# muzishen/IMAGDressing

Measured on AMD Instinct MI355X. Metric: 512x512 50-step images/sec (whole node), higher is better.
Workload: dtype bf16

## Files before the change

imagdressing_amd/_lib.py:

```python
from __future__ import annotations

import ctypes as C
import os

_HERE = os.path.dirname(os.path.abspath(__file__))
LIB_PATH = os.environ.get("IMD_LIB_PATH") or os.path.join(_HERE, "libimagdressing_hip.so")

ABI_VERSION = 9

u16p = C.POINTER(C.c_uint16)
f32p = C.POINTER(C.c_float)


class _Sized(C.Structure):

    def __init__(self, *args, **kw):
        super().__init__(*args, **kw)
        self.struct_bytes = C.sizeof(self)


class HeadsDest(C.Structure):
    _fields_ = [("ptr", C.c_void_p), ("kind", C.c_int), ("DP", C.c_int), ("L", C.c_int), ("scale", C.c_float)]


# ... 74 lines not shown

SYMBOLS = {
    "imd_abi_version": (C.c_int, []),
    "imd_last_error": (C.c_char_p, []),
    "imd_device_check": (C.c_int, [C.c_int]),
    "imd_conv_gemm": (C.c_int, [C.POINTER(ConvGemmParams), C.c_int, C.c_void_p]),
    "imd_conv_gemm_auto_cfg": (C.c_int, [C.c_int, C.c_int]),
    "imd_conv_gemm_auto_split": (C.c_int, [C.c_int, C.c_int, C.c_int, C.c_int]),
    "imd_attention": (C.c_int, [C.POINTER(AttnParams), C.c_void_p]),
    "imd_attention_dup_supported": (C.c_int, [C.c_int, C.c_int, C.c_int]),
    "imd_attention_phase_split_supported": (C.c_int, [C.c_int]),
    "imd_attention_fp8": (C.c_int, [C.POINTER(AttnParams), C.c_int, C.c_int, C.c_int, C.c_void_p]),
    "imd_attn_quantize_fp8": (C.c_int, [C.c_void_p, C.c_void_p, C.c_int, C.c_long, C.c_int, C.c_int, C.c_float, C.c_int, C.c_void_p]),
    "imd_set_tuning": (C.c_int, [C.c_int, C.c_int]),
    "imd_get_tuning": (C.c_int, [C.c_int]),
    "imd_attn_padded_dims": (C.c_int, [C.c_int, C.POINTER(C.c_int), C.POINTER(C.c_int)]),
    "imd_groupnorm": (C.c_int, [C.POINTER(GroupNormParams), C.c_void_p]),
    "imd_groupnorm_coeffs": (C.c_int, [C.POINTER(GroupNormParams), C.c_void_p, C.c_void_p, C.c_void_p]),
    "imd_conv_patch_supported": (C.c_int, [C.POINTER(ConvGemmParams)]),
    "imd_conv_patch2_supported": (C.c_int, [C.POINTER(ConvGemmParams)]),
    "imd_conv_patch3_supported": (C.c_int, [C.POINTER(ConvGemmParams)]),
    "imd_conv_patch4_supported": (C.c_int, [C.POINTER(ConvGemmParams)]),
    "imd_conv_img_supported": (C.c_int, [C.POINTER(ConvGemmParams)]),
    "imd_conv_patch_stats_parts": (C.c_int, [C.POINTER(ConvGemmParams)]),
    "imd_conv_gemm_stats_parts": (C.c_int, [C.POINTER(ConvGemmParams), C.c_int]),
    "imd_conv_gemm_gn_out_supported": (C.c_int, [C.POINTER(ConvGemmParams)]),
    "imd_row_linear_gn_in_supported": (C.c_int, [C.POINTER(ConvGemmParams), C.c_int]),
    "imd_gemm_dma_supported": (C.c_int, [C.POINTER(ConvGemmParams)]),
    "imd_row_linear": (C.c_int, [C.POINTER(ConvGemmParams), C.c_int, C.c_float, C.c_void_p]),
    "imd_row_linear_supported": (C.c_int, [C.POINTER(ConvGemmParams)]),
    "imd_ff_geglu": (C.c_int, [C.POINTER(FfParams), C.c_void_p]),
    "imd_text_xattn320": (C.c_int, [C.POINTER(XattnParams), C.c_void_p]),
    "imd_text_xattn320_supported": (C.c_int, [C.POINTER(XattnParams)]),
    "imd_groupnorm_workspace_floats": (C.c_int, [C.c_int, C.c_int, C.c_int, C.c_int]),
    "imd_layernorm": (C.c_int, [C.POINTER(LayerNormParams), C.c_void_p]),
    "imd_softmax_rows": (C.c_int, [C.c_void_p, C.c_int, C.c_void_p, C.c_int, C.c_int, C.c_int, C.c_int, C.c_void_p]),
    "imd_ddim_cfg_step": (C.c_int, [C.POINTER(DdimParams), C.c_void_p]),
    "imd_ddim_cfg_step_rows": (C.c_int, [C.POINTER(DdimParams), C.c_void_p, C.c_void_p]),
    "imd_timestep_embedding": (C.c_int, [C.c_void_p, C.c_void_p, C.c_int, C.c_int, C.c_void_p]),
    "imd_add": (C.c_int, [C.c_void_p, C.c_int, C.c_void_p, C.c_int, C.c_void_p, C.c_int, C.c_long, C.c_int, C.c_float, C.c_int, C.c_void_p]),
    "imd_embed_tokens": (C.c_int, [C.c_void_p, C.c_int, C.c_void_p, C.c_int, C.c_void_p, C.c_void_p, C.c_long, C.c_int, C.c_int, C.c_void_p]),
    "imd_vit_assemble": (C.c_int, [C.c_void_p, C.c_void_p, C.c_void_p, C.c_void_p, C.c_int, C.c_int, C.c_int, C.c_int, C.c_void_p]),
    "imd_lincomb": (C.c_int, [C.POINTER(C.c_void_p), C.POINTER(C.c_float), C.c_int, C.c_void_p, C.c_long, C.c_void_p]),
    "imd_copy2d": (C.c_int, [C.c_void_p, C.c_int, C.c_void_p, C.c_int, C.c_long, C.c_int, C.c_void_p]),
    "imd_concat2": (C.c_int, [C.c_void_p, C.c_int, C.c_void_p, C.c_int, C.c_void_p, C.c_void_p, C.c_long, C.c_long, C.c_int, C.c_void_p]),
    "imd_concat2_gn_stats": (C.c_int, [C.c_void_p, C.c_int, C.c_void_p, C.c_int, C.c_void_p, C.c_void_p, C.c_int, C.c_int, C.c_int, C.c_int,
                                       C.c_void_p, C.c_int, C.c_void_p]),
    "imd_groupnorm_parts": (C.c_int, [C.c_int, C.c_int, C.c_int]),
    "imd_f32_to_16": (C.c_int, [C.c_void_p, C.c_void_p, C.c_long, C.c_int, C.c_void_p]),
}

_lib = None


class ImdError(RuntimeError):
    pass


def load():
    global _lib
    if _lib is None:
        if not os.path.isfile(LIB_PATH):
            raise ImdError(
                f"{LIB_PATH} not found: build it with `python -c 'import __graft_entry__ as g; g.build()'` "
                "(or imagdressing_amd/csrc/build.sh).  imagdressing_amd has no CPU / torch fallback.")
        lib = C.CDLL(LIB_PATH)
# ... 13 lines not shown
```

imagdressing_amd/csrc/capi.cpp:

```cpp
#include <atomic>
#include <mutex>
#include <stdarg.h>
#include <stdio.h>
#include <string.h>

#include "imd_kernels.h"

namespace {
thread_local char g_err[512] = "";
}

int imd_set_error(const char* fmt, ...) {
    va_list ap;
    va_start(ap, fmt);
    vsnprintf(g_err, sizeof(g_err), fmt, ap);
    va_end(ap);
    return 1;
}

int imd_check_launch(const char* what) {
    hipError_t e = hipGetLastError();
    if (e != hipSuccess) return imd_set_error("%s: launch failed: %s", what, hipGetErrorString(e));
    return 0;
}
// ... 179 lines not shown
        IMD_REQUIRE(p->hC > 0 && p->hH > 0 && p->hD > 0 && p->hC == p->hH * p->hD && p->N % p->hC == 0 && p->N / p->hC <= 3 && p->hD % 8 == 0,
                    "row_linear: bad head split C=%d H=%d D=%d", p->hC, p->hH, p->hD);
        IMD_REQUIRE(!p->out_f32, "row_linear: head-split output excludes fp32 output");
    }
    IMD_REQUIRE(!ln || ln_eps > 0.f, "row_linear: LayerNorm needs eps > 0");
    if (p->K == 320 && p->N == 960 && p->mode == IMD_OUT_HEADS) {
        IMD_REQUIRE(p->gn_in_partial == nullptr, "row_linear: the fused q / k / v projection has no GroupNorm prologue (gn_in_*)");
        return imd_launch_row_qkv(*p, ln, ln_eps, (hipStream_t)stream);
    }
    if (p->K == 640) return imd_launch_row_linear_k640(*p, ln, ln_eps, (hipStream_t)stream);
    if (p->K == 1280) return imd_launch_row_linear_k1280(*p, ln, ln_eps, (hipStream_t)stream);
    return imd_launch_row_linear(*p, ln, ln_eps, (hipStream_t)stream);
}

int imd_ff_geglu(const imd_ff_params* p, void* stream) {
    IMD_REQUIRE(p != nullptr, "ff_geglu: null params");
    IMD_REQUIRE_SIZE(p, "ff_geglu");
    IMD_REQUIRE(p->x && p->w1 && p->b1 && p->w2 && p->b2 && p->out, "ff_geglu: null pointer");
    IMD_REQUIRE(!p->ln || p->ln_eps > 0.f, "ff_geglu: LayerNorm needs eps > 0");
    return imd_launch_ff_geglu(*p, (hipStream_t)stream);
}

int imd_text_xattn320_supported(const imd_xattn_params* p) {
    return (p && p->struct_bytes == sizeof(*p) && imd_text_xattn320_supported_of(*p)) ? 1 : 0;
}

int imd_text_xattn320(const imd_xattn_params* p, void* stream) {
    IMD_REQUIRE(p != nullptr, "text_xattn320: null params");
    IMD_REQUIRE_SIZE(p, "text_xattn320");
    IMD_REQUIRE(p->x && p->w && p->bq && p->bo && p->kv && p->out, "text_xattn320: null pointer");
    return imd_launch_text_xattn320(*p, (hipStream_t)stream);
}

int imd_layernorm(const imd_layernorm_params* p, void* stream) {
    IMD_REQUIRE(p != nullptr, "layernorm: null params");
    IMD_REQUIRE_SIZE(p, "layernorm");
    IMD_REQUIRE(p->x && p->y && p->gamma && p->beta, "layernorm: null pointer");
    return imd_launch_layernorm(*p, (hipStream_t)stream);
}

int imd_embed_tokens(const uint16_t* table, int vocab, const uint16_t* pos, int T, const int64_t* ids, uint16_t* out, long rows, int C,
                     int dtype, void* stream) {
    IMD_REQUIRE(table && pos && ids && out, "embed_tokens: null pointer");
    return imd_launch_embed_tokens(table, vocab, pos, T, ids, out, rows, C, dtype, (hipStream_t)stream);
}

int imd_vit_assemble(const uint16_t* patches, const uint16_t* cls, const uint16_t* pos, uint16_t* out, int B, int P, int C, int dtype,
                     void* stream) {
    IMD_REQUIRE(patches && cls && pos && out, "vit_assemble: null pointer");
    return imd_launch_vit_assemble(patches, cls, pos, out, B, P, C, dtype, (hipStream_t)stream);
}

int imd_lincomb(const float* const* xs, const float* coefs, int n, float* out, long numel, void* stream) {
    IMD_REQUIRE(xs && coefs && out, "lincomb: null pointer");
    return imd_launch_lincomb(xs, coefs, n, out, numel, (hipStream_t)stream);
}

int imd_softmax_rows(const float* s, int s_ld, uint16_t* p, int p_ld, int rows, int cols, int dtype, void* stream) {
    IMD_REQUIRE(s && p, "softmax_rows: null pointer");
    return imd_launch_softmax_rows(s, s_ld, p, p_ld, rows, cols, dtype, (hipStream_t)stream);
}

int imd_ddim_cfg_step(const imd_ddim_params* p, void* stream) {
    IMD_REQUIRE(p != nullptr, "ddim_cfg_step: null params");
    IMD_REQUIRE_SIZE(p, "ddim_cfg_step");
    IMD_REQUIRE(p->z && p->eps, "ddim_cfg_step: null pointer");
// ... 47 lines not shown
```

imagdressing_amd/csrc/conv_patch.hip:

```cpp
#include <type_traits>

#include "gemm_common.h"
#include "lds_dma.h"

namespace {

constexpr int TH = 8, TW = 16;
constexpr int PW = TW + 2, PH = TH + 2;
constexpr int NPIX = PH * PW;
constexpr int CK = 32;
constexpr int RSTR = CK * 2 + 16;
constexpr int BN = 128;
constexpr int A_BYTES = NPIX * RSTR;
constexpr int W_BYTES = BN * RSTR;
constexpr int MAIN_LDS = 2 * A_BYTES + 2 * W_BYTES;
constexpr int CLD = BN + 4;
constexpr int EROWS = 64;
constexpr int EPI_LDS = EROWS * CLD * 4;
constexpr int PATCH_LDS = MAIN_LDS > EPI_LDS ? MAIN_LDS : EPI_LDS;
constexpr int A_VECS = (NPIX * (CK / 8) + 255) / 256;
__device__ constexpr unsigned char kColPix[32] = {0, 1, 2, 3, 8, 9, 10, 11, 12, 13, 14, 15, 4, 5, 6, 7,
                                                  30, 31, 16, 17, 22, 23, 24, 25, 26, 27, 28, 29, 18, 19, 20, 21};
constexpr int W_VECS = BN * (CK / 8) / 256;

// ... 398 lines not shown
            float S = 0.f, Q = 0.f;
            for (int j = 0; j < CPR; ++j) {
                const int nj = n0 + 8 * j;
                if (nj >= p.N) break;
                const int gj = nj / cpg;
                if (gj == g || gj + 1 == g) {
                    const int o = (gj == g) ? 0 : 2;
                    for (int rl = 0; rl < 256 / CPR; ++rl) { S += red[(j + CPR * rl) * 4 + o]; Q += red[(j + CPR * rl) * 4 + o + 1]; }
                }
            }
            const int nparts = tiles_y * tiles_x * n_tiles;
            const int part = (ty * tiles_x + tx) * n_tiles + tile_n;
            float* dst = p.gn_stats_out + (((size_t)b * nparts + part) * G + g) * 2;
            dst[0] = S; dst[1] = Q;
        }
    }
    if (slab != nullptr && p.splitk_counters != nullptr) {
        if (splitk_last_arrival(p.splitk_counters, tile_id, p.split_k, tid)) {
            for (int ch = tid; ch < TH * TW * CPR; ch += 256) {
                const int q = ch / CPR, cc = (ch - q * CPR) * 8;
                const int oy = y0 + q / TW, ox = x0 + q % TW;
                const int n = n0 + cc;
                if (n >= p.N || oy >= H || ox >= W) continue;
                const int m = (b * H + oy) * W + ox;
                const int nv = (n + 8 <= p.N) ? 8 : 4;
                float v[8];
                splitk_sum8(p, m, n, nv, v);
                epilogue8<F16>(p, v, m, n, nv, HW);
            }
        }
    }
}

}

int imd_conv_patch_stats_parts_of(const ConvGemmParams& p) {
    if (!imd_conv_patch_supported(p) || p.split_k > 1 || p.out_f32 || p.gn_stats_groups <= 0 || p.gn_stats_groups > 64 ||
        p.N % p.gn_stats_groups || (p.N / p.gn_stats_groups) < 8)
        return 0;
    return ((p.Hout + TH - 1) / TH) * ((p.Wout + TW - 1) / TW) * ((p.N + BN - 1) / BN);
}

bool imd_conv_patch_supported(const ConvGemmParams& p) {
    const bool geom = p.ups ? (p.Hout == 2 * p.Hin && p.Wout == 2 * p.Win && p.gn_a == nullptr && !(g_gemm_flags & 512))
                            : (p.Hin == p.Hout && p.Win == p.Wout);
    return p.taps == 9 && p.stride == 1 && !p.pad_br_only && geom && p.Hout >= TH && p.Wout >= TW && (p.Cin % CK) == 0 &&
           p.mode == OUT_ROWMAJOR && p.act != ACT_GEGLU;
}

bool imd_conv_patch64_supported(const ConvGemmParams& p) {
    return imd_conv_patch_supported(p) && (p.Cin % 64) == 0 && p.gn_a == nullptr && !(g_gemm_flags & 512) && p.x_bytes < 0x80000000u && p.w_bytes < 0x80000000u;
}

int imd_launch_conv_patch64(const ConvGemmParams& p, hipStream_t s) {
    if (!imd_conv_patch64_supported(p)) return imd_set_error("conv_patch (128-byte rows): unsupported problem (needs 3x3 stride 1, H >= 8, W >= 16, Cin %% 64 == 0, operands < 2 GiB, no fused GroupNorm)");
    const bool h = p.dtype == IMD_DTYPE_F16;
    typedef void (*kern_t)(const ConvGemmParams);
    const kern_t kern = h ? conv3x3_patch_kernel<true, true, 64> : conv3x3_patch_kernel<false, true, 64>;
    if (int rc_attr = imd_lds_attr(reinterpret_cast<const void*>(kern), PD<64>::LDS, "conv_patch")) return rc_attr;
    const int B = p.M / (p.Hout * p.Wout);
    const long blocks = (long)B * ((p.Hout + TH - 1) / TH) * ((p.Wout + TW - 1) / TW) * ((p.N + BN - 1) / BN);
    hipLaunchKernelGGL(kern, dim3((unsigned)blocks, (unsigned)p.split_k), dim3(256), PD<64>::LDS, s, p);
    return imd_check_launch("conv_patch (128-byte rows)");
}

int imd_launch_conv_patch(const ConvGemmParams& p, hipStream_t s) {
// ... 15 lines not shown
```

imagdressing_amd/csrc/imd_kernels.h:

```cpp
#pragma once
#include <hip/hip_runtime.h>
#include <stdint.h>

#include "../../include/imagdressing_hip.h"

typedef uint16_t bf16_t;
typedef imd_heads_dest HeadsDest;
typedef imd_conv_gemm_params ConvGemmParams;
typedef imd_attn_params AttnParams;
typedef imd_groupnorm_params GroupNormParams;
typedef imd_layernorm_params LayerNormParams;
typedef imd_ddim_params DdimParams;

enum { ACT_NONE = IMD_ACT_NONE, ACT_SILU = IMD_ACT_SILU, ACT_GEGLU = IMD_ACT_GEGLU, ACT_GELU = IMD_ACT_GELU, ACT_QUICK_GELU = IMD_ACT_QUICK_GELU };
enum { OUT_ROWMAJOR = IMD_OUT_ROWMAJOR, OUT_HEADS = IMD_OUT_HEADS };

int imd_set_error(const char* fmt, ...);
int imd_check_launch(const char* what);
int imd_lds_attr(const void* kern, int bytes, const char* what);
int imd_cu_count8();

int imd_conv_gemm_choose_cfg(int M, int N);
int imd_conv_gemm_choose_split(int M, int N, int K, int cfg);
int imd_launch_conv_gemm(const ConvGemmParams& p, int cfg, hipStream_t s);
bool imd_conv_gemm_fill_extents(ConvGemmParams& p);
bool imd_conv_patch_supported(const ConvGemmParams& p);
bool imd_conv_patch2_supported(const ConvGemmParams& p);
int imd_launch_conv_patch2(const ConvGemmParams& p, hipStream_t s);
bool imd_conv_patch3_supported(const ConvGemmParams& p);
int imd_launch_conv_patch3(const ConvGemmParams& p, hipStream_t s);
bool imd_conv_patch4_supported(const ConvGemmParams& p);
int imd_launch_conv_patch4(const ConvGemmParams& p, hipStream_t s);
int imd_conv_patch3_stats_parts_of(const ConvGemmParams& p, int nw);
bool imd_conv_patch64_supported(const ConvGemmParams& p);
int imd_launch_conv_patch64(const ConvGemmParams& p, hipStream_t s);
bool imd_conv_img_supported(const ConvGemmParams& p);
int imd_launch_conv_img(const ConvGemmParams& p, hipStream_t s);
int imd_conv_patch_stats_parts_of(const ConvGemmParams& p);
int imd_conv_gemm_stats_parts_of(const ConvGemmParams& p, int cfg);
bool imd_conv_gemm_gn_out_supported_of(const ConvGemmParams& p, int cfg);
bool imd_row_linear_gn_in_supported_of(const ConvGemmParams& p, int cfg);
int imd_launch_conv_patch(const ConvGemmParams& p, hipStream_t s);
bool imd_row_linear_supported(const ConvGemmParams& p);
int imd_launch_row_linear(const ConvGemmParams& p, int ln, float ln_eps, hipStream_t s);
bool imd_row_linear_k640_supported(const ConvGemmParams& p);
int imd_launch_row_linear_k640(const ConvGemmParams& p, int ln, float ln_eps, hipStream_t s);
bool imd_row_linear_k1280_supported(const ConvGemmParams& p);
int imd_launch_row_linear_k1280(const ConvGemmParams& p, int ln, float ln_eps, hipStream_t s);
bool imd_row_qkv_supported(const ConvGemmParams& p);
int imd_launch_row_qkv(const ConvGemmParams& p, int ln, float ln_eps, hipStream_t s);
bool imd_gemm_dma_supported(const ConvGemmParams& p);
int imd_launch_gemm_dma(const ConvGemmParams& p, hipStream_t s);
int imd_launch_gemm_dma128(const ConvGemmParams& p, int stages, int bk, hipStream_t s);
int imd_launch_gemm_dma256(const ConvGemmParams& p, int form, hipStream_t s);
bool imd_conv_dma_supported(const ConvGemmParams& p);
int imd_launch_ff_geglu(const imd_ff_params& p, hipStream_t s);
bool imd_text_xattn320_supported_of(const imd_xattn_params& p);
int imd_launch_text_xattn320(const imd_xattn_params& p, hipStream_t s);
int imd_launch_attention(const AttnParams& p, hipStream_t s);
int imd_launch_attention_d40(const AttnParams& p, int variant, hipStream_t s);
int imd_launch_attention_fp8(const AttnParams& p, int eq, int ek, int ev, hipStream_t s);
int imd_launch_attn_quantize_fp8(const bf16_t* src, unsigned char* dst, int kind, long rows_or_groups, int LP, int exp2_scale,
                                 float pad_val, int dtype, hipStream_t s);
extern int g_attn_qw40;
extern int g_attn_xcd;
#ifdef IMD_ATTN_SWEEP
extern int g_attn_v80, g_attn_v160;
#endif
// ... 21 lines not shown
```

imagdressing_amd/ops.py:

```python
from __future__ import annotations

import functools
import ctypes as C
from typing import Dict, Optional, Sequence, Tuple

import torch

from . import _lib as L

ACT_NONE, ACT_SILU, ACT_GEGLU, ACT_GELU, ACT_QUICK_GELU = 0, 1, 2, 3, 4
bf16 = torch.bfloat16
f16 = torch.float16
DTYPE_CODE = {torch.bfloat16: 0, torch.float16: 1}


def _code(t: torch.Tensor, name: str = "tensor") -> int:
    try:
        return DTYPE_CODE[t.dtype]
    except KeyError:
        raise L.ImdError(f"{name}: expected a bfloat16 or float16 tensor, got {t.dtype}") from None


try:
    _raw_stream, _cur_dev = torch._C._cuda_getCurrentRawStream, torch._C._cuda_getDevice
# ... 575 lines not shown
    p.x, p.w, p.out = _dev(x, dt, "x"), _dev(packed["w"], dt, "w"), _dev(out, dt, "out")
    p.bq, p.bo, p.kv = _dev(packed["bq"], torch.float32, "bq"), _dev(packed["bo"], torch.float32, "bo"), _dev(kv_img, dt, "kv_img")
    p.M, p.C, p.heads, p.L = B * N, C_, XATTN_HEADS, int(Lk)
    p.rows_per_image, p.kv_bdiv, p.text_rows = N, int(kv_bdiv), kv_img.shape[0]
    p.x_ld = p.out_ld = C_
    p.q_scale = float(XATTN_D ** -0.5 * 1.4426950408889634 if q_scale is None else q_scale)
    p.ln_eps, p.dtype = float(ln_eps), _code(x, "x")
    _count("gemm_conv", 2 * 2.0 * B * N * C_ * C_)
    _count("attention", 4.0 * XATTN_HEADS * N * XATTN_D * B * Lk)
    L.check(L.load().imd_text_xattn320(C.byref(p), _stream()))
    return out


def conv2d_nhwc(x: torch.Tensor, w: torch.Tensor, bias=None, *, taps=9, stride=1, ups=False, rowvec=None,
                rowvec_stride=0, rowvec_off=0, res=None, out_scale=1.0, act=ACT_NONE, out_f32=False, cfg=-1, split_k=0, gn=None,
                pad_br_only=False, gn_stats_groups=0, gn_out=None, gn_in=None) -> torch.Tensor:
    B, H, W, Cin = x.shape
    Cout = w.shape[0]
    Hl, Wl = (2 * H, 2 * W) if ups else (H, W)
    Ho, Wo = ((Hl + stride - 1) // stride, (Wl + stride - 1) // stride)
    M = B * Ho * Wo
    out = conv_gemm(x, w, M=M, N=Cout, Cin=Cin, taps=taps, Hin=H, Win=W, Hout=Ho, Wout=Wo, stride=stride, ups=ups,
                    bias=bias, rowvec=rowvec, rowvec_stride=rowvec_stride, rowvec_off=rowvec_off, res=res, out_scale=out_scale, act=act,
                    out_f32=out_f32, cfg=cfg, split_k=split_k, gn=gn, pad_br_only=pad_br_only, gn_stats_groups=gn_stats_groups, gn_out=gn_out, gn_in=gn_in)
    r = out.view(B, Ho, Wo, -1)
    if getattr(out, "_imd_gn_applied", False):
        r._imd_gn_applied = True
    st = getattr(out, "_imd_gn_stats", None)
    if st is not None:
        r._imd_gn_stats = st
    return r


ATTN_EVENT_HOOK = None


FUSED_OUT_PROJ = _os.environ.get("IMD_FUSED_OUT_PROJ", "0") == "1"


def attention_proj_supported(H: int, N: int, D: int) -> bool:
    return D == 40 and H * D == 320 and N >= 512


_proj_cnt: Dict[Tuple, torch.Tensor] = {}


def proj_counters(n: int, device) -> torch.Tensor:
    key = (str(device), _stream())
    t = _proj_cnt.get(key)
    if t is None or t.numel() < n:
        t = torch.zeros(max(n, 4096), dtype=torch.int32, device=device)
        _proj_cnt[key] = t
    return t


def attention_dup_supported(H: int, N: int, D: int) -> bool:
    return bool(L.load().imd_attention_dup_supported(H, N, D))


ATTN_PHASE_SPLIT = _os.environ.get("IMD_ATTN_PHASE_SPLIT", "1") != "0"
ATTN_PHASE_SPLIT_MAX_N = int(_os.environ.get("IMD_ATTN_PHASE_SPLIT_MAX_N", "512"))


@functools.lru_cache(maxsize=None)
def attention_phase_split_supported(D: int) -> bool:
    return bool(L.load().imd_attention_phase_split_supported(D))
# ... 327 lines not shown
```

imagdressing_amd/unet.py:

```python
from __future__ import annotations

import math
from types import SimpleNamespace
from typing import Dict, List, Optional

import torch

from . import ops
from .hub import PretrainedMixin

FUSED_LN_CHANNELS = (320, 640, 1280)

bf16 = torch.bfloat16

SD15_CONFIG = dict(
    in_channels=4, out_channels=4, block_out_channels=(320, 640, 1280, 1280), layers_per_block=2,
    attention_head_dim=8, cross_attention_dim=768, norm_num_groups=32, sample_size=64,
    down_attn=(True, True, True, False), time_cond_proj_dim=None,
)


def _resnet_shapes(p, cin, cout, temb):
    s = {f"{p}.norm1.weight": (cin,), f"{p}.norm1.bias": (cin,),
         f"{p}.conv1.weight": (cout, cin, 3, 3), f"{p}.conv1.bias": (cout,),
# ... 115 lines not shown

def _f32(t, device):
    return t.detach().to(device=device, dtype=torch.float32).contiguous()


class LinearOp:

    def __init__(self, weight: torch.Tensor, bias: Optional[torch.Tensor], device, dtype=bf16):
        self.weight = weight.detach().to(device=device, dtype=dtype).contiguous()
        self.bias = None if bias is None else _f32(bias, device)
        self.out_features, self.in_features = self.weight.shape

    def __call__(self, x: torch.Tensor, **kw) -> torch.Tensor:
        x2 = x.to(self.weight.dtype).contiguous().view(-1, self.in_features)
        return ops.linear(x2, self.weight, self.bias, **kw).view(*x.shape[:-1], self.out_features)


class ConvOp:

    def __init__(self, weight: torch.Tensor, bias: Optional[torch.Tensor], device, dtype=bf16):
        cout, cin, kh, kw = weight.shape
        assert (kh, kw) in ((1, 1), (3, 3))
        cin_p = (cin + 7) // 8 * 8
        w = weight.detach().to(device=device, dtype=torch.float32).permute(0, 2, 3, 1)
        if cin_p != cin:
            w = torch.nn.functional.pad(w, (0, cin_p - cin))
        cout_p = (cout + 3) // 4 * 4
        self.weight = w.reshape(cout, kh * kw * cin_p).to(dtype).contiguous()
        self.bias = None if bias is None else _f32(bias, device)
        self.cin, self.cin_p, self.cout, self.taps = cin, cin_p, cout, kh * kw
        assert cout_p == cout, "output channels must be a multiple of 4"

    def __call__(self, x, **kw):
        return ops.conv2d_nhwc(x, self.weight, self.bias, taps=self.taps, **kw)


class NormParams:
    def __init__(self, sd, prefix, device):
        self.weight = _f32(sd[prefix + ".weight"], device)
        self.bias = _f32(sd[prefix + ".bias"], device)


class _Identity:
    def __call__(self, x):
        return x


class Attention:

    def __init__(self, sd, prefix, heads, device, dtype=bf16):
        self.heads = heads
        self.dtype = dtype
        self.to_q = LinearOp(sd[f"{prefix}.to_q.weight"], None, device, dtype)
        self.to_k = LinearOp(sd[f"{prefix}.to_k.weight"], None, device, dtype)
        self.to_v = LinearOp(sd[f"{prefix}.to_v.weight"], None, device, dtype)
        self.to_out = [LinearOp(sd[f"{prefix}.to_out.0.weight"], sd[f"{prefix}.to_out.0.bias"], device, dtype), _Identity()]
        self.query_dim = self.to_q.out_features
        self.is_cross = self.to_k.in_features != self.query_dim
        self.spatial_norm = None
        self.group_norm = None
        self.norm_cross = None
        self.residual_connection = False
        self.rescale_output_factor = 1.0
        self.processor = None

    def prepare_attention_mask(self, mask, *a, **k):
# ... 445 lines not shown
```

include/imagdressing_hip.h:

```cpp
#ifndef IMAGDRESSING_HIP_H
#define IMAGDRESSING_HIP_H

#include <stdint.h>

#ifdef __cplusplus
extern "C" {
#endif

#define IMD_ABI_VERSION 9

enum { IMD_ACT_NONE = 0, IMD_ACT_SILU = 1, IMD_ACT_GEGLU = 2, IMD_ACT_GELU = 3, IMD_ACT_QUICK_GELU = 4  };
enum { IMD_OUT_ROWMAJOR = 0, IMD_OUT_HEADS = 1 };
enum { IMD_DTYPE_BF16 = 0, IMD_DTYPE_F16 = 1 };

typedef struct imd_heads_dest {
    uint16_t* ptr;
    int kind;
    int DP;
    int L;
    float scale;
} imd_heads_dest;

#define IMD_TUNING_PER_CALL 0x5A000000
#define IMD_TUNING_TAG_MASK 0xFF000000u
// ... 149 lines not shown

int imd_attention(const imd_attn_params* p, void* stream);
int imd_attention_fp8(const imd_attn_params* p, int eq, int ek, int ev, void* stream);
int imd_attn_quantize_fp8(const uint16_t* src, uint8_t* dst, int kind, long count, int LP, int exp2_scale, float pad_val, int dtype,
                          void* stream);
int imd_row_linear_gn_in_supported(const imd_conv_gemm_params* p, int cfg);
int imd_conv_gemm_gn_out_supported(const imd_conv_gemm_params* p);
int imd_attention_dup_supported(int H, int N, int D);
int imd_attention_phase_split_supported(int D);
int imd_attn_padded_dims(int D, int* dpk, int* dpv);
int imd_set_tuning(int knob, int value);
int imd_get_tuning(int knob);

int imd_groupnorm(const imd_groupnorm_params* p, void* stream);
int imd_groupnorm_workspace_floats(int B, int HW, int C, int G);
int imd_groupnorm_coeffs(const imd_groupnorm_params* p, float* coef_a, float* coef_b, void* stream);
int imd_conv_patch_supported(const imd_conv_gemm_params* p);
int imd_conv_patch2_supported(const imd_conv_gemm_params* p);
int imd_conv_patch3_supported(const imd_conv_gemm_params* p);
int imd_conv_patch4_supported(const imd_conv_gemm_params* p);
int imd_conv_img_supported(const imd_conv_gemm_params* p);
int imd_conv_patch_stats_parts(const imd_conv_gemm_params* p);
int imd_conv_gemm_stats_parts(const imd_conv_gemm_params* p, int cfg);
int imd_gemm_dma_supported(const imd_conv_gemm_params* p);

int imd_row_linear(const imd_conv_gemm_params* p, int ln, float ln_eps, void* stream);
int imd_row_linear_supported(const imd_conv_gemm_params* p);

int imd_ff_geglu(const imd_ff_params* p, void* stream);

int imd_text_xattn320(const imd_xattn_params* p, void* stream);
int imd_text_xattn320_supported(const imd_xattn_params* p);

int imd_layernorm(const imd_layernorm_params* p, void* stream);
int imd_softmax_rows(const float* s, int s_ld, uint16_t* p, int p_ld, int rows, int cols, int dtype, void* stream);

int imd_ddim_cfg_step(const imd_ddim_params* p, void* stream);
int imd_ddim_cfg_step_rows(const imd_ddim_params* p, const float* guidance, void* stream);

int imd_timestep_embedding(const float* t, float* out, int B, int dim, void* stream);

int imd_add(const uint16_t* a, int a_ld, const uint16_t* b, int b_ld, uint16_t* out, int out_ld, long rows, int C, float b_scale, int dtype, void* stream);
int imd_embed_tokens(const uint16_t* table, int vocab, const uint16_t* pos, int T, const int64_t* ids, uint16_t* out, long rows, int C,
                     int dtype, void* stream);
int imd_vit_assemble(const uint16_t* patches, const uint16_t* cls, const uint16_t* pos, uint16_t* out, int B, int P, int C, int dtype,
                     void* stream);
int imd_lincomb(const float* const* xs, const float* coefs, int n, float* out, long numel, void* stream);
int imd_copy2d(const uint16_t* a, int a_ld, uint16_t* out, int out_ld, long rows, int C, void* stream);
int imd_concat2(const uint16_t* a, int Ca, const uint16_t* b, int Cb, const uint16_t* b_add, uint16_t* out, long rows, long b_rows, int dtype, void* stream);
int imd_concat2_gn_stats(const uint16_t* a, int Ca, const uint16_t* b, int Cb, const uint16_t* b_add, uint16_t* out, int B, int HW, int b_B, int G,
                         float* partial, int dtype, void* stream);
int imd_groupnorm_parts(int B, int HW, int C);
int imd_f32_to_16(const float* a, uint16_t* out, long n, int dtype, void* stream);

#ifdef __cplusplus
}
#endif
#endif
```

Before: 7.003.

## Add polyphase kernel for nearest-upsample followed by 3x3 conv

Adds a HIP kernel that computes nearest-2x upsample followed by a 3x3 convolution as four 2x2 sub-pixel phase convolutions on the low-resolution input, using pre-summed phase weights. This cuts MACs from 9 taps to 4 taps per output pixel and avoids reading the upsampled input. The UNet conv wrapper sends eligible upsample convs to it by default, based on grid-size and work-ratio heuristics. Costs are a host-side weight repack, cached per weight, and summing weights before rounding, which slightly changes numerics.

```diff
diff --git a/imagdressing_amd/_lib.py b/imagdressing_amd/_lib.py
--- a/imagdressing_amd/_lib.py
+++ b/imagdressing_amd/_lib.py
@@ -130,6 +130,8 @@
     "imd_ff_geglu": (C.c_int, [C.POINTER(FfParams), C.c_void_p]),
     "imd_text_xattn320": (C.c_int, [C.POINTER(XattnParams), C.c_void_p]),
     "imd_text_xattn320_supported": (C.c_int, [C.POINTER(XattnParams)]),
+    "imd_conv_ups_phase": (C.c_int, [C.POINTER(ConvGemmParams), C.c_void_p]),
+    "imd_conv_ups_phase_supported": (C.c_int, [C.POINTER(ConvGemmParams)]),
     "imd_groupnorm_workspace_floats": (C.c_int, [C.c_int, C.c_int, C.c_int, C.c_int]),
     "imd_layernorm": (C.c_int, [C.POINTER(LayerNormParams), C.c_void_p]),
     "imd_softmax_rows": (C.c_int, [C.c_void_p, C.c_int, C.c_void_p, C.c_int, C.c_int, C.c_int, C.c_int, C.c_void_p]),
diff --git a/imagdressing_amd/csrc/capi.cpp b/imagdressing_amd/csrc/capi.cpp
--- a/imagdressing_amd/csrc/capi.cpp
+++ b/imagdressing_amd/csrc/capi.cpp
@@ -235,6 +235,15 @@
     return imd_launch_text_xattn320(*p, (hipStream_t)stream);
 }
 
+int imd_conv_ups_phase_supported(const imd_conv_gemm_params* p) { return (sized(p) && imd_conv_ups_phase_supported_of(*p)) ? 1 : 0; }
+
+int imd_conv_ups_phase(const imd_conv_gemm_params* p, void* stream) {
+    IMD_REQUIRE(p != nullptr, "conv_ups_phase: null params");
+    IMD_REQUIRE_SIZE(p, "conv_ups_phase");
+    IMD_REQUIRE(p->x && p->w && p->out, "conv_ups_phase: null input / weight / output pointer");
+    return imd_launch_conv_ups_phase(*p, (hipStream_t)stream);
+}
+
 int imd_layernorm(const imd_layernorm_params* p, void* stream) {
     IMD_REQUIRE(p != nullptr, "layernorm: null params");
     IMD_REQUIRE_SIZE(p, "layernorm");
diff --git a/imagdressing_amd/csrc/conv_patch.hip b/imagdressing_amd/csrc/conv_patch.hip
--- a/imagdressing_amd/csrc/conv_patch.hip
+++ b/imagdressing_amd/csrc/conv_patch.hip
@@ -454,6 +454,242 @@
     }
 }
 
+template <bool F16>
+__global__ __launch_bounds__(256, 3) void conv_ups_phase_kernel(const ConvGemmParams p) {
+    using G = PD<32>;
+    using E = El<F16>;
+    constexpr int CKD = 32, NT = 4;
+    extern __shared__ __attribute__((aligned(16))) char smem[];
+
+    const int tid = threadIdx.x;
+    const int lane = tid & 63;
+    const int wave = tid >> 6;
+    const int wm0 = (wave >> 1) * 64;
+    const int wn0 = (wave & 1) * 64;
+    const int hi = lane >> 5, col = lane & 31;
+    const int cpix = kColPix[col];
+
+    const int H = p.Hin, W = p.Win;
+    const int tiles_x = (W + TW - 1) / TW, tiles_y = (H + TH - 1) / TH;
+    const int n_tiles = 4 * ((p.N + BN - 1) / BN);
+    int bid, tile_n;
+    xcd_tile_order(p.flags, (int)(gridDim.x / n_tiles), n_tiles, bid, tile_n);
+    const int phase = tile_n & 3, py = phase >> 1, px = phase & 1;
+    const int tx = bid % tiles_x; bid /= tiles_x;
+    const int ty = bid % tiles_y;
+    const int b = bid / tiles_y;
+    const int y0 = ty * TH, x0 = tx * TW, n0 = (tile_n >> 2) * BN;
+    const int nch = p.Cin / CKD;
+
+    const int wv = __builtin_amdgcn_readfirstlane(wave);
+    const uint32_t smem_base = (uint32_t)(uintptr_t)smem;
+    const v4i_t dx = raw_rsrc(p.x, p.x_bytes), dw = raw_rsrc(p.w, p.w_bytes);
+    constexpr uint32_t FAR = 0x80000000u;
+    uint32_t acur[G::APW], wcur[G::WPW], adst[G::APW], wdst[G::WPW];
+#pragma unroll
+    for (int i = 0; i < G::APW; ++i) {
+        const int slot = (wv * G::APW + i) * 64 + lane, pp = slot / G::LPR, piece = (slot % G::LPR) ^ G::swz(pp);
+        acur[i] = FAR;
+        if (pp < NPIX) {
+            const int iy = y0 - 1 + pp / PW, ix = x0 - 1 + pp % PW;
+            if ((unsigned)iy < (unsigned)H && (unsigned)ix < (unsigned)W)
+                acur[i] = (uint32_t)(((b * H + iy) * W + ix) * p.x_pix_stride + piece * 8) * 2u;
+        }
+        adst[i] = smem_base + (uint32_t)((wv * G::APW + i) * 1024);
+    }
+    const int Kp = NT * p.Cin;
+#pragma unroll
+    for (int i = 0; i < G::WPW; ++i) {
+        const int slot = (wv * G::WPW + i) * 64 + lane, row = slot / G::LPR, piece = (slot % G::LPR) ^ G::swz(row);
+        wcur[i] = (n0 + row < p.N) ? (uint32_t)((((size_t)phase * p.N + n0 + row) * Kp + piece * 8) * 2) : FAR;
+        wdst[i] = smem_base + (uint32_t)(2 * G::AB + (wv * G::WPW + i) * 1024);
+    }
+    const uint32_t w_tap = (uint32_t)(p.Cin * 2), w_chunk = (uint32_t)(CKD * 2) - (uint32_t)(NT - 1) * w_tap;
+    auto dma_patch = [&](auto buf_c) __attribute__((always_inline)) {
+#pragma unroll
+        for (int i = 0; i < G::APW; ++i) {
+            asm volatile("s_add_u32 m0, %1, %3\n\ts_nop 0\n\tbuffer_load_dwordx4 %0, %2, 0 offen lds"
+                         : : "v"(acur[i]), "s"(adst[i]), "s"(dx), "n"(decltype(buf_c)::value * G::AB) : "memory", "scc");
+            acur[i] += (uint32_t)(CKD * 2);
+        }
+    };
+    auto dma_w = [&](auto ring_c) __attribute__((always_inline)) {
+#pragma unroll
+        for (int i = 0; i < G::WPW; ++i) {
+            asm volatile("s_add_u32 m0, %1, %3\n\ts_nop 0\n\tbuffer_load_dwordx4 %0, %2, 0 offen lds"
+                         : : "v"(wcur[i]), "s"(wdst[i]), "s"(dw), "n"(decltype(ring_c)::value * G::WB) : "memory", "scc");
+            wcur[i] += w_tap;
+        }
+    };
+    int w_fr[2], xa[NT][2];
+#pragma unroll
+    for (int a = 0; a < 2; ++a) {
+        const int row = wn0 + a * 32 + col;
+        w_fr[a] = row * G::RB + ((hi ^ G::swz(row)) << 4);
+    }
+#pragma unroll
+    for (int bb = 0; bb < 2; ++bb) {
+        const int q = wm0 + bb * 32 + cpix, r0 = (q / TW) * PW + (q % TW);
+#pragma unroll
+        for (int t = 0; t < NT; ++t) {
+            const int rw = r0 + (py + (t >> 1)) * PW + (px + (t & 1));
+            xa[t][bb] = rw * G::RB + ((hi ^ G::swz(rw)) << 4);
+        }
+    }
+    const bool live = __builtin_amdgcn_readfirstlane((int)(n0 + (wv & 1) * 64 < p.N)) != 0;
+
+    f32x16 acc[2][2];
+#pragma unroll
+    for (int a = 0; a < 2; ++a)
+#pragma unroll
+        for (int bb = 0; bb < 2; ++bb)
+#pragma unroll
+            for (int r = 0; r < 16; ++r) acc[a][bb][r] = 0.f;
+
+    const std::integral_constant<int, 0> i0{}; const std::integral_constant<int, 1> i1{}; const std::integral_constant<int, 2> i2{};
+    dma_patch(i0);
+    dma_w(i0);
+    dma_w(i1);
+    dma_wait();
+    __syncthreads();
+    auto chunk = [&](auto j_c) __attribute__((always_inline)) {
+        constexpr int J = decltype(j_c)::value, AB = J & 1;
+        const char* As = smem + AB * G::AB;
+#pragma unroll
+        for (int t = 0; t < NT; ++t) {
+            const int cur = (NT * J + t) % 3, nxt = (NT * J + t + 2) % 3;
+            if (nxt == 0) dma_w(i0); else if (nxt == 1) dma_w(i1); else dma_w(i2);
+            if (t == 1) {
+#pragma unroll
+                for (int i = 0; i < G::WPW; ++i) wcur[i] += w_chunk - w_tap;
+                dma_patch(std::integral_constant<int, AB ^ 1>{});
+            }
+            if (live) {
+                const char* Wsm = smem + 2 * G::AB + cur * G::WB;
+                uint4 wf[2][2], xf[2][2];
+#pragma unroll
+                for (int kk = 0; kk < 2; ++kk) {
+#pragma unroll
+                    for (int a = 0; a < 2; ++a) wf[kk][a] = *reinterpret_cast<const uint4*>(Wsm + (w_fr[a] ^ (kk * 32)));
+#pragma unroll
+                    for (int bb = 0; bb < 2; ++bb) xf[kk][bb] = *reinterpret_cast<const uint4*>(As + (xa[t][bb] ^ (kk * 32)));
+                }
+#pragma unroll
+                for (int kk = 0; kk < 2; ++kk)
+#pragma unroll
+                    for (int a = 0; a < 2; ++a)
+#pragma unroll
+                        for (int bb = 0; bb < 2; ++bb) acc[a][bb] = E::mfma(wf[kk][a], xf[kk][bb], acc[a][bb]);
+            }
+            if (t == 1 || t == 2) dma_wait_keep_n<G::WPW + G::APW>(); else dma_wait_keep_n<G::WPW>();
+            __syncthreads();
+        }
+    };
+    {
+        int left = nch;
+#pragma unroll 1
+        for (;;) {
+            chunk(std::integral_constant<int, 0>{}); if (--left == 0) break;
+            chunk(std::integral_constant<int, 1>{}); if (--left == 0) break;
+            chunk(std::integral_constant<int, 2>{}); if (--left == 0) break;
+            chunk(std::integral_constant<int, 3>{}); if (--left == 0) break;
+            chunk(std::integral_constant<int, 4>{}); if (--left == 0) break;
+            chunk(std::integral_constant<int, 5>{}); if (--left == 0) break;
+        }
+    }
+    dma_wait();
+    __syncthreads();
+
+    float* Cs = reinterpret_cast<float*>(smem);
+    constexpr int CPR = BN / 8;
+    const int cc = (tid % CPR) * 8, n = n0 + cc;
+    const int nv = (n + 8 <= p.N) ? 8 : 4;
+    float4 b0 = make_float4(0, 0, 0, 0), b1 = b0;
+    if (p.bias != nullptr && n < p.N) {
+        b0 = *reinterpret_cast<const float4*>(p.bias + n);
+        if (nv == 8) b1 = *reinterpret_cast<const float4*>(p.bias + n + 4);
+    }
+    bf16_t* const outp = reinterpret_cast<bf16_t*>(p.out);
+#pragma unroll
+    for (int wr = 0; wr < 2; ++wr) {
+        if ((wave >> 1) == wr) {
+#pragma unroll
+            for (int bb = 0; bb < 2; ++bb)
+#pragma unroll
+                for (int a = 0; a < 2; ++a)
+#pragma unroll
+                    for (int j = 0; j < 4; ++j) {
+                        float* dst = Cs + (bb * 32 + cpix) * CLD + wn0 + a * 32 + 8 * j + 4 * hi;
+                        *reinterpret_cast<float4*>(dst) = make_float4(acc[a][bb][4 * j], acc[a][bb][4 * j + 1], acc[a][bb][4 * j + 2], acc[a][bb][4 * j + 3]);
+                    }
+        }
+        __syncthreads();
+#pragma unroll
+        for (int i = 0; i < 4; ++i) {
+            const int row = (tid + 256 * i) / CPR;
+            const int q = wr * EROWS + row;
+            const int sy = y0 + q / TW, sx = x0 + q % TW;
+            if (n >= p.N || sy >= H || sx >= W) continue;
+            const size_t m = ((size_t)(b * 2 * H + 2 * sy + py)) * (size_t)(2 * W) + (size_t)(2 * sx + px);
+            const float4 v0 = *reinterpret_cast<const float4*>(Cs + row * CLD + cc);
+            const float4 v1 = *reinterpret_cast<const float4*>(Cs + row * CLD + cc + 4);
+            const float v[8] = {v0.x + b0.x, v0.y + b0.y, v0.z + b0.z, v0.w + b0.w, v1.x + b1.x, v1.y + b1.y, v1.z + b1.z, v1.w + b1.w};
+            bf16_t* dst = outp + m * (size_t)p.out_ld + n;
+            if (nv == 8) *reinterpret_cast<uint4*>(dst) = pack8<F16>(v);
+            else *reinterpret_cast<uint2*>(dst) = make_uint2(E::pack2(v[0], v[1]), E::pack2(v[2], v[3]));
+        }
+        if (wr == 0) __syncthreads();
+    }
+}
+
+}
+
+static long ups_phase_units(int Hin, int Win) { return 16L * ((Hin + TH - 1) / TH) * ((Win + TW - 1) / TW); }
+static long ups_9tap_units(int Hout, int Wout) { return 9L * ((Hout + TH - 1) / TH) * ((Wout + TW - 1) / TW); }
+
+static bool ups_phase_can_run(const ConvGemmParams& p) {
+    if (!(p.taps == 9 && p.stride == 1 && p.ups && !p.pad_br_only && p.Hin > 0 && p.Win > 0 && p.Hout == 2 * p.Hin && p.Wout == 2 * p.Win)) return false;
+    if (p.Cin < CK || (p.Cin % CK) != 0 || p.K != 9 * p.Cin || p.N <= 0 || (p.N % 4) != 0 || p.M <= 0 || (p.M % (p.Hout * p.Wout)) != 0) return false;
+    if (p.x_pix_stride != p.Cin || p.out_ld != p.N || p.out_f32 || p.mode != OUT_ROWMAJOR) return false;
+    if (p.dtype != IMD_DTYPE_BF16 && p.dtype != IMD_DTYPE_F16) return false;
+    if (p.res != nullptr || p.res_rows != 0 || p.rowvec != nullptr || p.gn_a != nullptr || p.gn_b != nullptr || p.gn_stats_out != nullptr || p.gn_in_partial != nullptr ||
+        p.gn_out_gamma != nullptr || p.act != ACT_NONE || p.split_k > 1 || p.out_scale != 1.0f)
+        return false;
+    const size_t xb = (size_t)(p.M / 4) * p.Cin * 2, wb = (size_t)16 * p.N * p.Cin * 2, ob = (size_t)p.M * p.N * 2;
+    return xb < 0x80000000ull && wb < 0x80000000ull && ob < 0x80000000ull;
+}
+
+static long ups_phase_blocks(const ConvGemmParams& p) {
+    return (long)(p.M / (p.Hout * p.Wout)) * ((p.Hin + TH - 1) / TH) * ((p.Win + TW - 1) / TW) * 4 * ((p.N + BN - 1) / BN);
+}
+
+constexpr long UPS_PHASE_MIN_BLOCKS = 160;
+bool imd_conv_ups_phase_supported_of(const ConvGemmParams& p) {
+    if (!ups_phase_can_run(p)) return false;
+    if (ups_phase_blocks(p) < UPS_PHASE_MIN_BLOCKS) return false;
+    return 6 * ups_phase_units(p.Hin, p.Win) < 5 * ups_9tap_units(p.Hout, p.Wout);
+}
+
+int imd_launch_conv_ups_phase(const ConvGemmParams& p_in, hipStream_t s) {
+    if (!ups_phase_can_run(p_in))
+        return imd_set_error("conv_ups_phase: unsupported problem (needs 3x3 stride 1 with ups, Hout = 2 Hin, Wout = 2 Win, Cin %% 32 == 0, contiguous 16-bit input / output "
+                             "< 2 GiB, bias only)");
+    ConvGemmParams p = p_in;
+    const unsigned tag = (unsigned)p_in.flags & IMD_TUNING_TAG_MASK;
+    if (tag != 0 && tag != (unsigned)IMD_TUNING_PER_CALL)
+        return imd_set_error("conv_ups_phase: flags = 0x%x on entry is neither 0 nor IMD_TUNING_PER_CALL | bits (an uninitialised parameter block?)", (unsigned)p_in.flags);
+    const int gf = (tag == (unsigned)IMD_TUNING_PER_CALL) ? ((p_in.flags & 31) | (g_gemm_flags & ~31)) : g_gemm_flags;
+    p.flags = (gf & 4) ? (4 | (gf & 16)) : 0;
+    p.x_bytes = (uint32_t)((size_t)(p.M / 4) * p.Cin * 2);
+    p.w_bytes = (uint32_t)((size_t)16 * p.N * p.Cin * 2);
+    const bool h = p.dtype == IMD_DTYPE_F16;
+    typedef void (*kern_t)(const ConvGemmParams);
+    const kern_t kern = h ? conv_ups_phase_kernel<true> : conv_ups_phase_kernel<false>;
+    if (int rc_attr = imd_lds_attr(reinterpret_cast<const void*>(kern), PD<32>::LDS, "conv_ups_phase")) return rc_attr;
+    const long blocks = ups_phase_blocks(p);
+    if (blocks > 0x7fffffffL) return imd_set_error("conv_ups_phase: grid too large");
+    hipLaunchKernelGGL(kern, dim3((unsigned)blocks), dim3(256), PD<32>::LDS, s, p);
+    return imd_check_launch("conv_ups_phase");
 }
 
 int imd_conv_patch_stats_parts_of(const ConvGemmParams& p) {
diff --git a/imagdressing_amd/csrc/imd_kernels.h b/imagdressing_amd/csrc/imd_kernels.h
--- a/imagdressing_amd/csrc/imd_kernels.h
+++ b/imagdressing_amd/csrc/imd_kernels.h
@@ -34,6 +34,8 @@
 int imd_conv_patch3_stats_parts_of(const ConvGemmParams& p, int nw);
 bool imd_conv_patch64_supported(const ConvGemmParams& p);
 int imd_launch_conv_patch64(const ConvGemmParams& p, hipStream_t s);
+bool imd_conv_ups_phase_supported_of(const ConvGemmParams& p);
+int imd_launch_conv_ups_phase(const ConvGemmParams& p, hipStream_t s);
 bool imd_conv_img_supported(const ConvGemmParams& p);
 int imd_launch_conv_img(const ConvGemmParams& p, hipStream_t s);
 int imd_conv_patch_stats_parts_of(const ConvGemmParams& p);
diff --git a/imagdressing_amd/ops.py b/imagdressing_amd/ops.py
--- a/imagdressing_amd/ops.py
+++ b/imagdressing_amd/ops.py
@@ -631,6 +631,101 @@
     return r
 
 
+UPS_PHASE = _os.environ.get("IMD_UPS_PHASE", "1") != "0"
+UPS_PHASE_TAPS = (((0,), (1, 2)), ((0, 1), (2,)))
+UPS_PHASE_CFG = "ups_phase"
+_UPS_W: Dict[Tuple, tuple] = {}
+_UPS_OK: Dict[Tuple, bool] = {}
+_clear_hooks.append(_UPS_W.clear)
+_clear_hooks.append(_UPS_OK.clear)
+
+
+def _pack_upsample_phase(w: torch.Tensor, dtype=None) -> torch.Tensor:
+    N, Cp = w.shape[0], w.shape[1] // 9
+    acc_dt = torch.float32 if w.dtype in DTYPE_CODE else w.dtype
+    w9 = w.to(acc_dt).view(N, 3, 3, Cp)
+    out = torch.zeros(4, N, 4, Cp, dtype=acc_dt, device=w.device)
+    for py in range(2):
+        for px in range(2):
+            for dy in range(2):
+                for dx in range(2):
+                    for ky in UPS_PHASE_TAPS[py][dy]:
+                        for kx in UPS_PHASE_TAPS[px][dx]:
+                            out[2 * py + px, :, 2 * dy + dx] += w9[:, ky, kx]
+    return out.to(w.dtype if dtype is None else dtype).contiguous()
+
+
+def pack_upsample_phase(w: torch.Tensor, dtype=None) -> torch.Tensor:
+    if w.dim() != 2 or w.shape[1] % 9:
+        raise L.ImdError(f"pack_upsample_phase: expected a packed 3x3 weight [Cout, 9 * Cin], got {tuple(w.shape)}")
+    key = (w.data_ptr(), w._version, w.dtype, str(w.device), tuple(w.shape), dtype)
+    ent = _UPS_W.get(key)
+    if ent is None:
+        if len(_UPS_W) > 64:
+            _UPS_W.clear()
+        ent = _UPS_W[key] = (w, _pack_upsample_phase(w, dtype))
+    return ent[1]
+
+
+def _ups_phase_block(shape, N: int, dtype):
+    B, H, W, Cin = shape
+    p = L.ConvGemmParams()
+    p.flags = _gemm_call_flags()
+    p.dtype, p.M, p.N, p.K, p.Cin, p.taps = DTYPE_CODE[dtype], 4 * B * H * W, N, 9 * Cin, Cin, 9
+    p.Hin, p.Win, p.Hout, p.Wout, p.stride, p.ups = H, W, 2 * H, 2 * W, 1, 1
+    p.x_pix_stride, p.out_ld, p.res_ld, p.out_scale, p.split_k = Cin, N, N, 1.0, 1
+    return p
+
+
+def conv_ups_phase_supported(x: torch.Tensor, w: torch.Tensor, bias=None) -> bool:
+    if x.dim() != 4 or w.dim() != 2 or w.shape[1] != 9 * x.shape[3] or x.dtype not in DTYPE_CODE or w.dtype != x.dtype or not x.is_contiguous():
+        return False
+    key = (tuple(x.shape), w.shape[0], x.dtype)
+    ok = _UPS_OK.get(key)
+    if ok is None:
+        ok = bool(L.load().imd_conv_ups_phase_supported(C.byref(_ups_phase_block(x.shape, w.shape[0], x.dtype))))
+        if len(_UPS_OK) < 4096:
+            _UPS_OK[key] = ok
+    return ok
+
+
+def conv_ups_phase(x: torch.Tensor, w: torch.Tensor, bias=None, *, out: Optional[torch.Tensor] = None,
+                   phase_weights: Optional[torch.Tensor] = None) -> torch.Tensor:
+    ensure_device(x.device)
+    B, H, W, Cin = x.shape
+    N = w.shape[0]
+    M, K = 4 * B * H * W, 9 * Cin
+    dt = x.dtype
+    if w.dim() != 2 or tuple(w.shape) != (N, K) or w.dtype != dt:
+        raise L.ImdError(f"conv_ups_phase: expected a packed 3x3 weight [{N}, {K}] of {dt}, got {tuple(w.shape)} {w.dtype}")
+    wp = pack_upsample_phase(w) if phase_weights is None else phase_weights
+    if tuple(wp.shape) != (4, N, 4, Cin):
+        raise L.ImdError(f"conv_ups_phase: phase weights must be [4, {N}, 4, {Cin}], got {tuple(wp.shape)}")
+    if out is None:
+        out = torch.empty((B, 2 * H, 2 * W, N), dtype=dt, device=x.device)
+    elif out.numel() != M * N:
+        raise L.ImdError(f"conv_ups_phase: out has {out.numel()} elements, expected {M * N}")
+    p = _ups_phase_block(x.shape, N, dt)
+    p.x, p.w, p.out = _dev(x, dt, "x"), _dev(wp, dt, "phase weights"), _dev(out, dt, "out")
+    p.bias = None if bias is None else _dev(bias, torch.float32, "bias")
+    _count("gemm_conv", 2.0 * M * N * K)
+    if GEMM_TRACE is not None:
+        GEMM_TRACE.append(dict(M=M, N=N, K=K, Cin=Cin, taps=9, Hin=H, Win=W, Hout=2 * H, Wout=2 * W, stride=1, ups=1, splittable=True, dtype=str(x.dtype),
+                               bias=bias is not None, rowvec=False, rowvec_stride=0, res=False, res_rows=0, act=ACT_NONE, out_f32=False, heads=None,
+                               gn_stats_groups=0, x_pix_stride=Cin, out_scale=1.0, pad_br_only=False, out_ld=N, res_ld=N, gn=False, gn_in=False, gn_out=False,
+                               ups_phase=True))
+    lib = L.load()
+    if GEMM_EVENT_HOOK is not None:
+        e0, e1 = torch.cuda.Event(enable_timing=True), torch.cuda.Event(enable_timing=True)
+        e0.record()
+        L.check(lib.imd_conv_ups_phase(C.byref(p), _stream()))
+        e1.record()
+        GEMM_EVENT_HOOK.setdefault((f"{M},{N},{K},9,1,1|{2 * H}x{2 * W}", UPS_PHASE_CFG, 1), []).append((e0, e1))
+    else:
+        L.check(lib.imd_conv_ups_phase(C.byref(p), _stream()))
+    return out.view(B, 2 * H, 2 * W, N)
+
+
 ATTN_EVENT_HOOK = None
 
 
diff --git a/imagdressing_amd/unet.py b/imagdressing_amd/unet.py
--- a/imagdressing_amd/unet.py
+++ b/imagdressing_amd/unet.py
@@ -171,6 +171,8 @@
         assert cout_p == cout, "output channels must be a multiple of 4"
 
     def __call__(self, x, **kw):
+        if ops.UPS_PHASE and self.taps == 9 and kw == {"ups": True} and ops.conv_ups_phase_supported(x, self.weight, self.bias):
+            return ops.conv_ups_phase(x, self.weight, self.bias)
         return ops.conv2d_nhwc(x, self.weight, self.bias, taps=self.taps, **kw)
 
 
diff --git a/include/imagdressing_hip.h b/include/imagdressing_hip.h
--- a/include/imagdressing_hip.h
+++ b/include/imagdressing_hip.h
@@ -205,6 +205,9 @@
 int imd_text_xattn320(const imd_xattn_params* p, void* stream);
 int imd_text_xattn320_supported(const imd_xattn_params* p);
 
+int imd_conv_ups_phase(const imd_conv_gemm_params* p, void* stream);
+int imd_conv_ups_phase_supported(const imd_conv_gemm_params* p);
+
 int imd_layernorm(const imd_layernorm_params* p, void* stream);
 int imd_softmax_rows(const float* s, int s_ld, uint16_t* p, int p_ld, int rows, int cols, int dtype, void* stream);
 
```

Result: faster. 7.144, median of 6 (+2.0%).
